# ToughStoneX/Self-Supervised-MVS

Hardware: AMD Instinct MI355X
Metric: depth-samples/sec (N=3, 640x512, D=192) (higher is better)
Workload: dtype f32

## Files before the change

### self-supervised-mvs_amd/_lib.py

```python
from __future__ import annotations

import ctypes as C
import os

_HERE = os.path.dirname(os.path.abspath(__file__))
LIB_PATH = os.path.join(_HERE, "libmvs_hip.so")

_f = C.c_void_p
_i = C.c_int
_ll = C.c_longlong
_s = C.c_void_p
_fl = C.c_float

class MvsUnetBlock(C.Structure):
    _fields_ = [("transposed", _i), ("stride", _i), ("src", _i), ("skip", _i), ("eps", _fl), ("momentum", _fl),
                ("cin", _i), ("cout", _i), ("d", _i), ("h", _i), ("w", _i)]


class MvsFeatBlock(C.Structure):
    _fields_ = [("cin", _i), ("cout", _i), ("ks", _i), ("stride", _i), ("eps", _fl), ("momentum", _fl), ("w_channels_last", _i),
                ("h", _i), ("w", _i)]


_pp = C.POINTER(C.c_void_p)
# ... 74 lines not shown
}

OP_CONV_FWD, OP_CONV_DGRAD, OP_CONV_WGRAD, OP_CONVT_FWD, OP_CONVT_DGRAD, OP_CONVT_WGRAD = range(6)


class MvsLib:

    def __init__(self, path: str = LIB_PATH, device_type: str = "cuda"):
        if not os.path.exists(path):
            raise RuntimeError(
                "libmvs_hip.so not found at %s -- build it with `python __graft_entry__.py` "
                "(hipcc --offload-arch=gfx950); there is no CPU / PyTorch fallback for the hot path" % path)
        self.path = path
        self.device_type = device_type
        self.cdll = C.CDLL(path)
        self.profiler = None
        for name, (res, args) in SIGNATURES.items():
            fn = getattr(self.cdll, name)
            fn.restype = res
            fn.argtypes = args
            setattr(self, "_" + name, fn)

    def call(self, name: str, *args, tag="", tstream=None):
        prof = self.profiler
        if prof is not None and (prof.names is None or name in prof.names):
            if not isinstance(tag, str):
                tag = tag[0] % tuple(tag[1:])
            if prof.wants(name, tag):
                import torch
                ev0, ev1 = torch.cuda.Event(enable_timing=True), torch.cuda.Event(enable_timing=True)
                ev0.record(tstream)
                rc = getattr(self, "_" + name)(*args)
                ev1.record(tstream)
                prof.add(name, tag, ev0, ev1)
                if rc != 0:
                    self._raise(name, rc)
                return
        rc = getattr(self, "_" + name)(*args)
        if rc != 0:
            self._raise(name, rc)

    def _raise(self, name, rc):
        msg = self._mvs_last_error().decode("utf-8", "replace")
        if rc in (-1, -2, -4):
            raise ValueError("%s failed (%d): %s" % (name, rc, msg))
        raise RuntimeError("%s failed (%d): %s" % (name, rc, msg))

    def raw(self, name: str, *args):
        return getattr(self, "_" + name)(*args)


_INSTANCE = None

DEFAULT_TUNING = {"k8": 7, "xcd": 1, "side_pre": 1, "conv_pers": 1, "conv_pers_min": 1024, "conv_pers_nw": 8, "wgrad_pers": 1, "conv_small": 1, "tr2pw": 1, "sweep_bwd": 0, "wgrad_small": 0, "wgrad_groups": 768, "wgrad8_groups": 192, "wgrad8_gs": 2, "wgrad8_nch": 2, "cout1_h4": 1, "wgrad2d_batch": 2048}


def get() -> MvsLib:
    global _INSTANCE
    if _INSTANCE is None:
        _INSTANCE = MvsLib()
        for item in filter(None, os.environ.get("MVS_TUNING", "").split(",")):
            key, _, val = item.partition("=")
            DEFAULT_TUNING[key.strip()] = int(val)
            _INSTANCE.call("mvs_set_tuning", key.strip().encode(), int(val))
    return _INSTANCE


class KernelTimer:

    def __init__(self, only=None, names=None):
        self.only = only
        self.names = names
        self.events = {}

    def wants(self, name, tag):
        return self.only is None or name in self.only or tag in self.only

    def add(self, name, tag, ev0, ev1):
        self.events.setdefault((name, tag), []).append((ev0, ev1))

    _REG_NAMES = frozenset(("mvs_conv3d_fwd", "mvs_convT3d_fwd", "mvs_conv3d_dgrad", "mvs_convT3d_dgrad", "mvs_conv3d_wgrad", "mvs_convT3d_wgrad",
                            "mvs_bn_relu_fwd_slots", "mvs_bn_relu_bwd_slots", "mvs_bn_bwd_reduce_slots", "mvs_conv3d_pack_weights_batch"))

    def allows_c_entry(self, lib, blocks):
        if self.names is None:
            return False
        hit = self.names & self._REG_NAMES
        if not hit:
            return True
        if not hit <= {"mvs_conv3d_wgrad", "mvs_convT3d_wgrad"} or self.only is None:
            return False
        want = [t for t in self.only if isinstance(t, str) and t.startswith("wgrad")]
        found = []
        for i, (transposed, cin, cout, stride, dims) in enumerate(blocks):
            tag = "%s:%d>%d:s%d:%dx%dx%dx%d" % (("wgradT" if transposed else "wgrad", cin, cout, stride) + tuple(dims))
            if tag in want:
                found.append((i, "mvs_convT3d_wgrad" if transposed else "mvs_conv3d_wgrad", tag))
        if len(found) != 1 or len(want) != 1:
            return False
        owner = getattr(lib, "_unet_timer", None)
        if owner is not self:
            if owner is not None:
                owner._harvest()
                owner._c = None
            lib.raw("mvs_unet_time_read", (C.c_float * 1024)(), 1024)
            lib.raw("mvs_unet_time_wgrad", found[0][0])
            lib._unet_timer = self
# ... 37 lines not shown
```

### self-supervised-mvs_amd/csrc/conv3d.hip

```cpp
#include "mvs_rt.h"
#include "conv_map.h"

int g_conv_cout1_d4 = 2;

extern int g_conv_split, g_conv_small, g_conv_small_wgs, g_conv_tr2pw;

#include "conv_args.h"

__device__ __forceinline__ void conv_pack_weights_item(const float* __restrict__ w, float* __restrict__ wp, int geom, int CC,
                                                       int Cin, int Cout, int NB, int layout, int flip, int idx) {
    const int j = idx & 3, lane = (idx >> 2) & 63;
    const int nb = (idx >> 8) % NB, kk = (idx >> 8) / NB;
    const int co = nb * 16 + (lane & 15);
    int ks, chunk = 0, cls = 0;
    if (geom == GEOM_TR2_PW) {
        int k0 = 0;
        for (cls = 0; cls < 4; ++cls) {
            int n = tr2p_ntaps(cls) * CC / 16;
            if (kk < k0 + n) break;
            k0 += n;
        }
        ks = kk - k0;
        const int kf = 16 * ks + 4 * (lane >> 4) + j;
        const int tp = kf / CC, cip = kf % CC, n = lane & 15, pw = n >> 3, cop = n & 7;
// ... 293 lines not shown
                const int f = wave * MB + mb;
                const int qd = qd0 + f / G::TQH, qh = qh0 + f % G::TQH;
                if (qd >= a.QD || qh >= a.QH) continue;
                const int od = qd * G::OS + pd_of(cls), oh = qh * G::OS + ph_of(cls);
#pragma unroll
                for (int r = 0; r < 4; ++r) {
                    const int qw = qw0 + 4 * g + r;
                    if (qw >= a.QW) continue;
                    const int ow = qw * G::OS + pw_of(cls);
                    const size_t obase = ((((size_t)b * a.Do + od) * a.Ho + oh) * a.Wo + ow) * a.Cout;
#pragma unroll
                    for (int nb = 0; nb < NB; ++nb) {
                        const int co = G::PW ? (l15 & 7) : (nb0 + nb) * 16 + l15;
                        if (co >= a.Cout) continue;
                        float v = acc[mb][nb][r];
                        float sv1 = v, sv2 = v * v;
                        if (a.scale) v = v * a.scale[co] + a.shift[co];
                        else if (a.shift) v = v + a.shift[co];
                        if (a.relu) v = fmaxf(v, 0.f);
                        if (SIDE && a.skip) v += SIDE_PRE ? skp[SIDE_PRE ? mb : 0][r][nb] : sk[e][r][nb];
                        if (SIDE && a.bn_raw) {
                            const float rw = SIDE_PRE ? rwp[SIDE_PRE ? mb : 0][r][nb] : rwv[e][r][nb];
                            sv1 = (rw * bsc[nb] + bsh[nb] > 0.f) ? v : 0.f;
                            sv2 = sv1 * ((rw - bmu[nb]) * bis[nb]);
                        }
                        st1[nb] += sv1;
                        st2[nb] += sv2;
                        a.y[obase + co] = v;
                    }
                }
            }
        }
    }

    if (a.slots) {
#pragma unroll
        for (int nb = 0; nb < NB; ++nb) {
            float s1 = st1[nb], s2 = st2[nb];
            s1 += __shfl_xor(s1, 16); s1 += __shfl_xor(s1, 32);
            s2 += __shfl_xor(s2, 16); s2 += __shfl_xor(s2, 32);
            if (G::PW) { s1 += __shfl_xor(s1, 8); s2 += __shfl_xor(s2, 8); }
            if (lane < 16) {
                red[((wave * NB + nb) * 16 + lane) * 2 + 0] = s1;
                red[((wave * NB + nb) * 16 + lane) * 2 + 1] = s2;
            }
        }
        __syncthreads();
        if (tid < 2 * NB * 16) {
            const int stat = tid / (NB * 16), n = tid % (NB * 16);
            if (nb0 * 16 + n < a.Cout) {
                float s = 0.f;
                for (int w = 0; w < 4; ++w) s += red[(w * NB * 16 + n) * 2 + stat];
                MVS_GLOBAL_ATOMIC_ADD_F64(a.slots + ((size_t)(blockIdx.x & (a.nslots - 1)) * 2 + stat) * a.Cout + nb0 * 16 + n, (double)s);
            }
        }
    }
}

template <int COUT, int VPT>
__global__ __launch_bounds__(256) void conv_cin1_kernel(const float* __restrict__ x, const float* __restrict__ wt,
                                                        float* __restrict__ y, int B, int D, int H, int W,
                                                        const float* __restrict__ bn_raw, const float* __restrict__ bn_stats,
                                                        double* __restrict__ slots, int nslots) {
    __shared__ float red[4 * 2 * COUT];
    const size_t total = (size_t)B * D * H * W;
    float sv[2 * COUT];
#pragma unroll
    for (int k = 0; k < 2 * COUT; ++k) sv[k] = 0.f;
#pragma unroll 1
    for (int it = 0; it < VPT; ++it) {
        const size_t v0 = ((size_t)blockIdx.x * VPT + it) * 256 + threadIdx.x;
        const bool live = v0 < total;
        const size_t v = live ? v0 : total - 1;
        const int w_ = (int)(v % W), h_ = (int)((v / W) % H), d_ = (int)((v / ((size_t)W * H)) % D);
        float4 rwq[COUT / 4];
#pragma unroll
        for (int q = 0; q < COUT / 4; ++q)
            rwq[q] = (slots && live) ? *reinterpret_cast<const float4*>(bn_raw + v * COUT + 4 * q) : make_float4(0.f, 0.f, 0.f, 0.f);
        int dofs[3], hofs[3], wofs[3];
        bool vd[3], vh[3], vw[3];
#pragma unroll
        for (int i = 0; i < 3; ++i) {
            const int d = d_ + i - 1, h = h_ + i - 1, w = w_ + i - 1;
            vd[i] = d >= 0 && d < D; vh[i] = h >= 0 && h < H; vw[i] = w >= 0 && w < W;
            dofs[i] = (min(max(d, 0), D - 1) - d_) * H * W;
            hofs[i] = (min(max(h, 0), H - 1) - h_) * W;
            wofs[i] = min(max(w, 0), W - 1) - w_;
        }
        const float* __restrict__ xc = x + v;
        float xv[27];
#pragma unroll
        for (int t = 0; t < 27; ++t) xv[t] = xc[dofs[t / 9] + hofs[(t / 3) % 3] + wofs[t % 3]];
        float acc[COUT];
#pragma unroll
        for (int c = 0; c < COUT; ++c) acc[c] = 0.f;
#pragma unroll
        for (int t = 0; t < 27; ++t) {
            const float xt = (vd[t / 9] && vh[(t / 3) % 3] && vw[t % 3]) ? xv[t] : 0.f;
#pragma unroll
            for (int c = 0; c < COUT; ++c) acc[c] = fmaf(xt, wt[t * COUT + c], acc[c]);
        }
        if (live) {
#pragma unroll
            for (int c = 0; c < COUT; c += 4)
                *reinterpret_cast<float4*>(y + v * COUT + c) = make_float4(acc[c], acc[c + 1], acc[c + 2], acc[c + 3]);
        }
// ... 824 lines not shown
                            const int bl = lane >> 2;
                            const int idx = BC ? ((4 * tg + (lane >> 4)) * 16 + (lane & 15)) * 8 + 4 * h + r
                                               : ((4 * tg + (bl >> 2)) * 16 + 4 * (bl & 3) + r) * 8 + (lane & 3) + 4 * h;
                            if (wv == 0) xt[idx] = acc[ch][tg][h][r];
                            else xt[idx] += acc[ch][tg][h][r];
                        }
            }
            __syncthreads();
        }
        for (int i = tid; i < 28 * 16 * 8; i += 256) {
            const int co = i & 7, cx = (i >> 3) & 15, tap = tapmap[i >> 7];
            if (tap < 27) a.part[(((size_t)blockIdx.x * 27 + tap) * a.CX + (chunk0 + ch) * 16 + cx) * 8 + co] = xt[i];
        }
    }
}

__global__ __launch_bounds__(256) void conv_wgrad_reduce_wide_kernel(const float* __restrict__ part, int nparts, int CX, int CG,
                                                                     float* __restrict__ gw) {
    __shared__ float red[16][17];
    const int n = 27 * CX * CG;
    const int el = threadIdx.x & 15, slice = threadIdx.x >> 4;
    const int e = blockIdx.x * 16 + el;
    const size_t stride = (size_t)n;
    float s0 = 0.f, s1 = 0.f, s2 = 0.f, s3 = 0.f;
    if (e < n) {
        int p = slice;
        for (; p + 48 < nparts; p += 64) {
            const float a0 = part[(size_t)p * stride + e], a1 = part[(size_t)(p + 16) * stride + e];
            const float a2 = part[(size_t)(p + 32) * stride + e], a3 = part[(size_t)(p + 48) * stride + e];
            s0 += a0; s1 += a1; s2 += a2; s3 += a3;
        }
        for (; p < nparts; p += 16) s0 += part[(size_t)p * stride + e];
    }
    red[slice][el] = (s0 + s1) + (s2 + s3);
    __syncthreads();
    if (slice == 0 && e < n) {
        float t = 0.f;
#pragma unroll
        for (int k = 0; k < 16; ++k) t += red[k][el];
        const int cg = e % CG, cx = (e / CG) % CX, tap = e / (CG * CX);
        gw[((size_t)cg * CX + cx) * 27 + tap] = t;
    }
}

static int pick_cc(int geom, int cin) {
    if (geom == GEOM_TR2) return cin;
    if (geom == GEOM_S2) return 8;
    return (cin % 16 == 0) ? 16 : 8;
}

int g_conv_cc_wide = 0;
int g_conv_cin1_vpt = 1;
static int pick_cc_k(int geom, int kgeom, int cin) {
    if (g_conv_cc_wide) {
        if (kgeom == GEOM_S1_SMALL && (cin == 32 || cin == 64)) return cin;
        if (kgeom == GEOM_S2_SMALL && (cin == 16 || cin == 32)) return cin;
    }
    return pick_cc(geom, cin);
}

static size_t packed_floats(int geom, int cin, int cout) {
    const int cc = pick_cc(geom, cin);
    int nb = mvs_cdiv(cout, 16);
    if (nb == 3) nb = 4;
    return (size_t)total_ksteps(geom, cin, cc) * nb * 256;
}

int g_conv_split = 1;
int g_conv_tr2pw = 1;
int g_conv_small_wgs = 384;
int g_conv_small = 1;
int g_conv_c8 = 7;
int g_conv_wgrad_groups = 768;
int g_conv_cout1_h4 = 1;
int g_conv_wgrad8_groups = 192;
int g_conv_wgrad8_nch = 2;
int g_conv_wgrad_small = 0;
int g_conv_side_pre = 1;
int g_conv_pers = 1;
int g_conv_pers_min_wgs = 1024;
int g_conv_wgrad_pers = 1;
bool conv_wgrad_pers_serves(int geom, int CX, int CG);
int run_conv_wgrad_pers(int geom, const WgradArgs& a, int max_groups, hipStream_t st);
bool conv_c8_wgrad_gs_serves(int geom, int CX, int CG);
int run_conv_c8_wgrad_gs(const WgradArgs& a, int max_groups, int waves, hipStream_t st);
int g_conv_wgrad8_gs = 2;
bool conv_pers_serves(int geom, int cin, int cout);
int run_conv_pers(int geom, const ConvArgs& a, hipStream_t st);
bool conv_x3_serves(int geom, const ConvArgs& a);
int run_conv_x3(const ConvArgs& a, const float* w, int wlayout, int flip, hipStream_t st);
bool conv_x3_fwd_serves(int geom, const ConvArgs& a);
int run_conv_x3_fwd(const ConvArgs& a, const float* w, int wlayout, int flip, float* ws, hipStream_t st);
extern int g_conv_x3;
int g_conv_xcd = 1;

template <int GEOM, int CC>
static int launch_igemm_nb(const ConvArgs& a, int NB, int nblocks, hipStream_t st) {
    dim3 grid(nblocks, a.nb_total / NB), block(256);
    if (a.skip || a.bn_raw) {
        switch (NB) {
            case 1:
                if (g_conv_side_pre) MVS_LAUNCH((conv_igemm_kernel<GEOM, CC, 1, 2>), grid, block, 0, st, a);
                else MVS_LAUNCH((conv_igemm_kernel<GEOM, CC, 1, 1>), grid, block, 0, st, a);
                break;
            case 2: MVS_LAUNCH((conv_igemm_kernel<GEOM, CC, 2, 1>), grid, block, 0, st, a); break;
            case 4: MVS_LAUNCH((conv_igemm_kernel<GEOM, CC, 4, 1>), grid, block, 0, st, a); break;
            default: mvs_set_error("conv igemm: Cout tile count %d unsupported", NB); return MVS_ERR_UNSUPPORTED;
        }
        return mvs_check_launch("conv_igemm");
    }
    switch (NB) {
        case 1: MVS_LAUNCH((conv_igemm_kernel<GEOM, CC, 1, 0>), grid, block, 0, st, a); break;
        case 2: MVS_LAUNCH((conv_igemm_kernel<GEOM, CC, 2, 0>), grid, block, 0, st, a); break;
        case 4: MVS_LAUNCH((conv_igemm_kernel<GEOM, CC, 4, 0>), grid, block, 0, st, a); break;
        default: mvs_set_error("conv igemm: Cout tile count %d unsupported", NB); return MVS_ERR_UNSUPPORTED;
    }
    return mvs_check_launch("conv_igemm");
}

static void igemm_tiling(int geom, int B, int QD, int QH, int QW, int cout, int& kgeom, int& NB, int& nblocks) {
    const int nb_total = mvs_cdiv(cout, 16) == 3 ? 4 : mvs_cdiv(cout, 16);
    nblocks = B * mvs_cdiv(QD, geom_tqd(geom)) * mvs_cdiv(QH, geom_tqh(geom)) * mvs_cdiv(QW, 16);
    NB = nb_total;
    if (g_conv_split && nblocks < 512 && NB > 1) NB = 1;
    kgeom = geom;
    const long thr = (long)g_conv_small_wgs * (geom == GEOM_S2 ? 24 : (geom == GEOM_S1 ? 3 : 1));
    if (g_conv_small == 2 || (g_conv_small == 1 && (long)nblocks * (nb_total / NB) < thr)) {
        kgeom = geom + GEOM_S1_SMALL;
        nblocks = B * mvs_cdiv(QD, geom_tqd(kgeom)) * mvs_cdiv(QH, geom_tqh(kgeom)) * mvs_cdiv(QW, 16);
    }
}

struct Epilogue {
    const float* scale; const float* shift; const float* skip; int relu;
    double* slots; int nslots;
    const float* bn_raw; const float* bn_stats;
};

struct IgemmPlan {
    int geom, wlayout, flip, B, Di, Hi, Wi, cin, cout;
    bool cin1;
};
enum { MVS_OP_CONV_FWD = 0, MVS_OP_CONV_DGRAD = 1, MVS_OP_CONV_WGRAD = 2,
       MVS_OP_CONVT_FWD = 3, MVS_OP_CONVT_DGRAD = 4, MVS_OP_CONVT_WGRAD = 5 };

static int check_stride(int stride, int D, int H, int W, const char* what) {
    MVS_REQUIRE(stride == 1 || stride == 2, MVS_ERR_UNSUPPORTED, "%s: stride must be 1 or 2, got %d", what, stride);
    MVS_REQUIRE(D > 0 && H > 0 && W > 0, MVS_ERR_SHAPE, "%s: bad spatial shape %dx%dx%d", what, D, H, W);
    return MVS_OK;
}

static int plan_for(int op, int B, int D, int H, int W, int Cin, int Cout, int stride, IgemmPlan& p, const char* what) {
    int rc = check_stride(stride, D, H, W, what);
    if (rc) return rc;
    MVS_REQUIRE(B > 0 && (long long)B * D * H * W * (stride == 2 ? 8 : 1) < (1LL << 31), MVS_ERR_SHAPE,
                "%s: %d x %d x %d x %d voxels do not fit the kernels' 32-bit voxel indices", what, B, D, H, W);
    p = {};
    p.B = B; p.cin1 = false;
    switch (op) {
        case MVS_OP_CONV_FWD:
            p.geom = stride == 2 ? GEOM_S2 : GEOM_S1; p.wlayout = WL_OIK; p.flip = 0;
            p.Di = D; p.Hi = H; p.Wi = W; p.cin = Cin; p.cout = Cout;
            return MVS_OK;
        case MVS_OP_CONV_DGRAD:
            p.cin = Cout; p.cout = Cin; p.wlayout = WL_IOK;
            if (stride == 1) {
                p.geom = GEOM_S1; p.flip = 1; p.Di = D; p.Hi = H; p.Wi = W;
                p.cin1 = Cout == 1;
            } else {
                MVS_REQUIRE(D % 2 == 0 && H % 2 == 0 && W % 2 == 0, MVS_ERR_SHAPE, "%s stride 2: D,H,W must be even", what);
                p.geom = GEOM_TR2; p.flip = 0; p.Di = D / 2; p.Hi = H / 2; p.Wi = W / 2;
            }
            return MVS_OK;
        case MVS_OP_CONVT_FWD:
            p.wlayout = WL_IOK; p.Di = D; p.Hi = H; p.Wi = W; p.cin = Cin; p.cout = Cout;
            if (stride == 1) { p.geom = GEOM_S1; p.flip = 1; } else { p.geom = GEOM_TR2; p.flip = 0; }
            return MVS_OK;
        case MVS_OP_CONVT_DGRAD:
            p.wlayout = WL_OIK; p.flip = 0; p.cin = Cout; p.cout = Cin;
            if (stride == 1) { p.geom = GEOM_S1; p.Di = D; p.Hi = H; p.Wi = W; }
            else { p.geom = GEOM_S2; p.Di = 2 * D; p.Hi = 2 * H; p.Wi = 2 * W; }
            return MVS_OK;
        default:
            mvs_set_error("%s: op %d has no weight image", what, op);
            return MVS_ERR_UNSUPPORTED;
    }
}

static void plan_grid(const IgemmPlan& p, int& QD, int& QH, int& QW) {
    if (p.geom == GEOM_S2) { QD = (p.Di - 1) / 2 + 1; QH = (p.Hi - 1) / 2 + 1; QW = (p.Wi - 1) / 2 + 1; }
    else { QD = p.Di; QH = p.Hi; QW = p.Wi; }
}
static bool plan_is_c8(const IgemmPlan& p, const Epilogue* ep) {
    return (g_conv_c8 & 3) && p.geom == GEOM_S1 && p.cout == 8 && (p.cin == 8 || p.cin == 16 || p.cin == 32) && !(ep && ep->bn_raw);
}
static bool plan_is_cout1(const IgemmPlan& p, const Epilogue* ep) {
    return p.geom == GEOM_S1 && p.cout == 1 && p.wlayout == WL_OIK && !p.flip && (p.cin == 8 || p.cin == 16) &&
           !(ep && (ep->slots || ep->bn_raw));
}

static int plan_pack(const IgemmPlan& p, const float* w, float* ws, PackItem& it) {
    it = {};
    it.w = w; it.wp = ws; it.kind = -1;
    if (p.cin1) {
        MVS_REQUIRE(p.cout == 8 || p.cout == 16, MVS_ERR_UNSUPPORTED, "conv3d_dgrad(Cout=1): Cin must be 8 or 16, got %d", p.cout);
        it.kind = 1; it.Cout = p.cout; it.total = 27 * p.cout;
        return MVS_OK;
    }
    MVS_REQUIRE(p.cin == 8 || p.cin == 16 || p.cin == 32 || p.cin == 64, MVS_ERR_UNSUPPORTED,
                "conv igemm: input channels must be 8/16/32/64, got %d", p.cin);
    MVS_REQUIRE(p.cout >= 1 && p.cout <= 64, MVS_ERR_UNSUPPORTED, "conv igemm: output channels must be <= 64, got %d", p.cout);
    MVS_REQUIRE(!(p.geom == GEOM_TR2 && p.cin < 16), MVS_ERR_UNSUPPORTED, "transposed stride-2 conv needs >= 16 input channels");
    int QD, QH, QW, kgeom, NB, nblocks;
    plan_grid(p, QD, QH, QW);
    igemm_tiling(p.geom, p.B, QD, QH, QW, p.cout, kgeom, NB, nblocks);
    const int cc = pick_cc_k(p.geom, kgeom, p.cin);
    const int nb_total = mvs_cdiv(p.cout, 16) == 3 ? 4 : mvs_cdiv(p.cout, 16);
    const int pgeom = (kgeom == GEOM_TR2 && cc == 16 && p.cout == 8 && g_conv_tr2pw) ? GEOM_TR2_PW : p.geom;
    it.kind = 0; it.geom = pgeom; it.CC = cc; it.Cin = p.cin; it.Cout = p.cout; it.NB = nb_total; it.layout = p.wlayout; it.flip = p.flip;
    it.total = (int)((size_t)total_ksteps(pgeom, p.cin, cc) * nb_total * 256);
    return MVS_OK;
}

static int launch_pack(const PackItem* items, int n, hipStream_t st) {
    for (int i0 = 0; i0 < n; i0 += MVS_PACK_BATCH_MAX) {
        PackBatch pb = {};
        int m = 0, maxtotal = 0;
        for (int i = i0; i < n && m < MVS_PACK_BATCH_MAX; ++i) {
            if (items[i].kind < 0) continue;
            pb.it[m++] = items[i];
            if (items[i].total > maxtotal) maxtotal = items[i].total;
        }
        if (m == 0) continue;
        MVS_LAUNCH(conv_pack_batch_kernel, dim3(mvs_cdiv(maxtotal, 256), m), dim3(256), 0, st, pb);
    }
    return mvs_check_launch("conv_pack_weights");
}

static int run_igemm(const IgemmPlan& p, const float* in, const float* wsrc, float* out, float* ws, const Epilogue& ep,
                     int ws_packed, hipStream_t st) {
    MVS_REQUIRE(in && wsrc && out && ws, MVS_ERR_NULL, "conv: null pointer argument");
    MVS_REQUIRE(!ep.slots || (ep.nslots >= 1 && ep.nslots <= 256 && (ep.nslots & (ep.nslots - 1)) == 0), MVS_ERR_SHAPE,
                "conv: statistic slot count must be a power of two <= 256, got %d", ep.nslots);
    MVS_REQUIRE(!ep.bn_raw || (ep.bn_stats && ep.slots), MVS_ERR_NULL, "conv: bn_raw needs bn_stats and slots");
    const int geom = p.geom, B = p.B, cin = p.cin, cout = p.cout;
    ConvArgs a = {};
    a.x = in; a.y = out; a.B = B; a.Di = p.Di; a.Hi = p.Hi; a.Wi = p.Wi; a.Cin = cin; a.Cout = cout;
    a.scale = ep.scale; a.shift = ep.shift; a.skip = ep.skip; a.relu = ep.relu;
    a.slots = ep.slots; a.nslots = ep.nslots; a.bn_raw = ep.bn_raw; a.bn_stats = ep.bn_stats;
    plan_grid(p, a.QD, a.QH, a.QW);
    if (geom == GEOM_S1) { a.Do = p.Di; a.Ho = p.Hi; a.Wo = p.Wi; }
    else if (geom == GEOM_S2) { a.Do = a.QD; a.Ho = a.QH; a.Wo = a.QW; }
    else { a.Do = 2 * p.Di; a.Ho = 2 * p.Hi; a.Wo = 2 * p.Wi; }
    a.ntd = mvs_cdiv(a.QD, geom_tqd(geom)); a.nth = mvs_cdiv(a.QH, geom_tqh(geom)); a.ntw = mvs_cdiv(a.QW, 16);
    if ((g_conv_x3 & 1) && conv_x3_serves(geom, a)) return run_conv_x3(a, wsrc, p.wlayout, p.flip, st);
    if ((g_conv_x3 & 2) && conv_x3_fwd_serves(geom, a)) return run_conv_x3_fwd(a, wsrc, p.wlayout, p.flip, ws, st);
    if (plan_is_c8(p, &ep)) {
        const int ntl = B * a.ntd * a.nth * a.ntw;
        const int nbc = ntl < 512 ? ntl : 512;
        if (cin == 32) MVS_LAUNCH((conv_c8_fwd_bc_kernel<16, 2>), dim3(nbc), dim3(256), 0, st, a, wsrc, p.wlayout, p.flip, g_conv_xcd);
        else if (cin == 16) MVS_LAUNCH((conv_c8_fwd_bc_kernel<16, 1>), dim3(nbc), dim3(256), 0, st, a, wsrc, p.wlayout, p.flip, g_conv_xcd);
        else MVS_LAUNCH((conv_c8_fwd_bc_kernel<8, 1>), dim3(nbc), dim3(256), 0, st, a, wsrc, p.wlayout, p.flip, g_conv_xcd);
        return mvs_check_launch("conv_c8_fwd_bc");
    }
    int nblocks = B * a.ntd * a.nth * a.ntw;
    if (plan_is_cout1(p, &ep)) {
        if (cin == 8 && g_conv_cout1_h4) {
            a.ntd = mvs_cdiv(a.QD, CO1_TD); a.nth = mvs_cdiv(a.QH, CO1_TH); a.ntw = mvs_cdiv(a.QW, CO1_TW);
            MVS_LAUNCH(conv_cout1_h4_kernel, dim3(B * a.ntd * a.nth * a.ntw), dim3(256), 0, st, a, wsrc);
        } else if (cin == 8) MVS_LAUNCH((conv_cout1_kernel<8>), dim3(nblocks), dim3(256), 0, st, a, wsrc);
        else MVS_LAUNCH((conv_cout1_kernel<16>), dim3(nblocks), dim3(256), 0, st, a, wsrc);
        return mvs_check_launch("conv_cout1");
    }
    int NB, kgeom;
    a.nb_total = mvs_cdiv(cout, 16) == 3 ? 4 : mvs_cdiv(cout, 16);
    igemm_tiling(geom, B, a.QD, a.QH, a.QW, cout, kgeom, NB, nblocks);
    const int cc = pick_cc_k(geom, kgeom, cin);
    a.ntd = mvs_cdiv(a.QD, geom_tqd(kgeom)); a.nth = mvs_cdiv(a.QH, geom_tqh(kgeom));
    if (!ws_packed) {
        PackItem it;
        int rc = plan_pack(p, wsrc, ws, it);
        if (rc) return rc;
        rc = launch_pack(&it, 1, st);
        if (rc) return rc;
    } else {
        MVS_REQUIRE(cin == 8 || cin == 16 || cin == 32 || cin == 64, MVS_ERR_UNSUPPORTED, "conv igemm: input channels must be 8/16/32/64, got %d", cin);
        MVS_REQUIRE(cout >= 1 && cout <= 64, MVS_ERR_UNSUPPORTED, "conv igemm: output channels must be <= 64, got %d", cout);
        MVS_REQUIRE(!(geom == GEOM_TR2 && cin < 16), MVS_ERR_UNSUPPORTED, "transposed stride-2 conv needs >= 16 input channels");
    }
    a.wp = ws;
    if (g_conv_pers && conv_pers_serves(geom, cin, cout) && (long)nblocks * (a.nb_total / NB) >= g_conv_pers_min_wgs) {
        a.ntd = mvs_cdiv(a.QD, geom_tqd(geom)); a.nth = mvs_cdiv(a.QH, geom_tqh(geom));
        return run_conv_pers(geom, a, st);
    }
    if ((g_conv_pers & 1) && kgeom == GEOM_TR2 && cc == 16 && cout == 8 && g_conv_tr2pw && conv_pers_serves(GEOM_TR2_PW, cin, cout) &&
        nblocks >= g_conv_pers_min_wgs)
        return run_conv_pers(GEOM_TR2_PW, a, st);
    if (kgeom == GEOM_S1) return cc == 16 ? launch_igemm_nb<GEOM_S1, 16>(a, NB, nblocks, st)
                                          : launch_igemm_nb<GEOM_S1, 8>(a, NB, nblocks, st);
    if (kgeom == GEOM_S2) return launch_igemm_nb<GEOM_S2, 8>(a, NB, nblocks, st);
    if (kgeom == GEOM_S1_SMALL) {
        if (cc == 64) return launch_igemm_nb<GEOM_S1_SMALL, 64>(a, NB, nblocks, st);
        if (cc == 32) return launch_igemm_nb<GEOM_S1_SMALL, 32>(a, NB, nblocks, st);
        return cc == 16 ? launch_igemm_nb<GEOM_S1_SMALL, 16>(a, NB, nblocks, st) : launch_igemm_nb<GEOM_S1_SMALL, 8>(a, NB, nblocks, st);
    }
    if (kgeom == GEOM_S2_SMALL) {
        if (cc == 32) return launch_igemm_nb<GEOM_S2_SMALL, 32>(a, NB, nblocks, st);
        if (cc == 16) return launch_igemm_nb<GEOM_S2_SMALL, 16>(a, NB, nblocks, st);
        return launch_igemm_nb<GEOM_S2_SMALL, 8>(a, NB, nblocks, st);
    }
    if (kgeom == GEOM_TR2_SMALL) {
        if (cc == 16) return launch_igemm_nb<GEOM_TR2_SMALL, 16>(a, NB, nblocks, st);
        if (cc == 32) return launch_igemm_nb<GEOM_TR2_SMALL, 32>(a, NB, nblocks, st);
        return launch_igemm_nb<GEOM_TR2_SMALL, 64>(a, NB, nblocks, st);
    }
    if (cc == 16 && cout == 8 && g_conv_tr2pw) return launch_igemm_nb<GEOM_TR2_PW, 16>(a, NB, nblocks, st);
    if (cc == 16) return launch_igemm_nb<GEOM_TR2, 16>(a, NB, nblocks, st);
    if (cc == 32) return launch_igemm_nb<GEOM_TR2, 32>(a, NB, nblocks, st);
    return launch_igemm_nb<GEOM_TR2, 64>(a, NB, nblocks, st);
}

static int run_cin1(const IgemmPlan& p, const float* gy, const float* w, float* gx, float* ws, const Epilogue& ep, int ws_packed,
                    hipStream_t st) {
    MVS_REQUIRE(gy && w && gx && ws, MVS_ERR_NULL, "conv3d_dgrad: null pointer argument");
    MVS_REQUIRE(!ep.skip, MVS_ERR_UNSUPPORTED, "conv3d_dgrad: the Cout = 1 input gradient takes no summand");
    MVS_REQUIRE(!ep.bn_raw || (ep.bn_stats && ep.slots), MVS_ERR_NULL, "conv3d_dgrad: bn_raw needs bn_stats and slots");
    MVS_REQUIRE(!ep.slots || (ep.bn_raw && ep.nslots >= 1 && ep.nslots <= 256 && (ep.nslots & (ep.nslots - 1)) == 0), MVS_ERR_SHAPE,
                "conv3d_dgrad: bad statistic slots");
    const int C = p.cout;
    if (!ws_packed) {
        PackItem it;
        int rc = plan_pack(p, w, ws, it);
        if (rc) return rc;
        rc = launch_pack(&it, 1, st);
        if (rc) return rc;
    } else {
        MVS_REQUIRE(C == 8 || C == 16, MVS_ERR_UNSUPPORTED, "conv3d_dgrad(Cout=1): Cin must be 8 or 16, got %d", C);
    }
    const size_t total = (size_t)p.B * p.Di * p.Hi * p.Wi;
    const int vpt = (g_conv_cin1_vpt == 5 || (g_conv_cin1_vpt == 4 && total >= (size_t)1 << 20)) ? 4 : 1;
    dim3 grid((unsigned)((total + 256 * vpt - 1) / (256 * vpt)));
    if (C == 8 && vpt == 4) MVS_LAUNCH((conv_cin1_kernel<8, 4>), grid, dim3(256), 0, st, gy, (const float*)ws, gx, p.B, p.Di, p.Hi, p.Wi, ep.bn_raw, ep.bn_stats, ep.slots, ep.nslots);
    else if (C == 8) MVS_LAUNCH((conv_cin1_kernel<8, 1>), grid, dim3(256), 0, st, gy, (const float*)ws, gx, p.B, p.Di, p.Hi, p.Wi, ep.bn_raw, ep.bn_stats, ep.slots, ep.nslots);
// ... 205 lines not shown
```

### self-supervised-mvs_amd/csrc/conv_map.h

```cpp
#pragma once

#if defined(__HIPCC__) || defined(MVS_CPU_EMUL)
#define MVS_HD __host__ __device__
#else
#define MVS_HD
#endif

enum { GEOM_S1 = 0, GEOM_S2 = 1, GEOM_TR2 = 2,
       GEOM_S1_SMALL = 3, GEOM_S2_SMALL = 4, GEOM_TR2_SMALL = 5,
       GEOM_TR2_PW = 6,
       GEOM_S1_DP = 7 };
enum { WL_OIK = 0, WL_IOK = 1 };

template <int GEOM>
struct ConvGeom;
template <>
struct ConvGeom<GEOM_S1> {
    static constexpr bool PW = false;
    static constexpr int BASE = GEOM_S1;
    static constexpr int TQD = 4, TQH = 4, TQW = 16, MB = 4;
    static constexpr int IS = 1, OS = 1, NCLS = 1, PAD = 1;
    static constexpr int RD = TQD + 2, RH = TQH + 2, RW = TQW + 2;
};
template <>
struct ConvGeom<GEOM_S1_DP> {
    static constexpr bool PW = false;
    static constexpr int BASE = GEOM_S1;
    static constexpr int TQD = 4, TQH = 4, TQW = 16, MB = 4;
    static constexpr int IS = 1, OS = 1, NCLS = 1, PAD = 1;
    static constexpr int RD = TQD + 2, RH = TQH + 2, RW = TQW + 2;
};
template <>
struct ConvGeom<GEOM_S2> {
    static constexpr bool PW = false;
    static constexpr int BASE = GEOM_S2;
    static constexpr int TQD = 2, TQH = 4, TQW = 16, MB = 2;
    static constexpr int IS = 2, OS = 1, NCLS = 1, PAD = 1;
    static constexpr int RD = 2 * TQD + 1, RH = 2 * TQH + 1, RW = 2 * TQW + 1;
};
template <>
struct ConvGeom<GEOM_TR2_PW> {
    static constexpr int BASE = GEOM_TR2;
    static constexpr bool PW = true;
    static constexpr int TQD = 4, TQH = 4, TQW = 16, MB = 4;
    static constexpr int IS = 1, OS = 2, NCLS = 4, PAD = 0;
    static constexpr int RD = TQD + 1, RH = TQH + 1, RW = TQW + 1;
};
template <>
struct ConvGeom<GEOM_TR2> {
    static constexpr bool PW = false;
    static constexpr int BASE = GEOM_TR2;
    static constexpr int TQD = 4, TQH = 4, TQW = 16, MB = 4;
    static constexpr int IS = 1, OS = 2, NCLS = 8, PAD = 0;
    static constexpr int RD = TQD + 1, RH = TQH + 1, RW = TQW + 1;
};
template <>
struct ConvGeom<GEOM_S1_SMALL> {
    static constexpr bool PW = false;
    static constexpr int BASE = GEOM_S1;
    static constexpr int TQD = 2, TQH = 2, TQW = 16, MB = 1;
    static constexpr int IS = 1, OS = 1, NCLS = 1, PAD = 1;
    static constexpr int RD = TQD + 2, RH = TQH + 2, RW = TQW + 2;
};
template <>
// ... 58 lines not shown
```

### self-supervised-mvs_amd/csrc/plane_sweep.hip

```cpp
#include <stdlib.h>
#include <string.h>
#include "mvs_rt.h"

#include <type_traits>
#include "plane_sweep_common.h"

template <int C, int NS_T>
__global__ __launch_bounds__(256) void plane_sweep_variance_fwd_kernel(SweepArgs a) {
    constexpr int QUADS = C / 4;
    constexpr int TW = Tile<C>::TW, TH = Tile<C>::TH;
    const int NS = NS_T > 0 ? NS_T : a.NS;
    const int tid = threadIdx.x;
    const int q = tid % QUADS, pl = tid / QUADS;
    const int x = (blockIdx.x % a.tiles_x) * TW + pl % TW, y = (blockIdx.x / a.tiles_x) * TH + pl / TW;
    const int b = blockIdx.z;
    if (x >= a.W || y >= a.H) return;
    const int HW = a.H * a.W, pix = y * a.W + x;
    const int d0 = blockIdx.y * a.dslab;
    const int d1 = min(a.D, d0 + a.dslab);
    const float xf = (float)x, yf = (float)y;
    const size_t fbase = (size_t)b * HW * C + 4 * q;
    const float4 r = ld4(a.ref + fbase + (size_t)pix * C);
    const float4 r2 = make_float4(r.x * r.x, r.y * r.y, r.z * r.z, r.w * r.w);
    const float inv_n = 1.0f / (float)(NS + 1);
// ... 1110 lines not shown
#pragma unroll
            for (int j = 0; j < 4; ++j) {
                jx0[j] = s_win[j][s][0]; jy0[j] = s_win[j][s][1];
                jw[j] = s_win[j][s][4] ? s_win[j][s][2] : 0; jh[j] = s_win[j][s][3];
            }
            float* gp = a.gsrc[s] + (size_t)b * HW * C;
            for (int i = tid; i < uw * uh * C; i += 256) {
                const int c = i % C, t = i / C;
                const int txl = ux0 + t % uw, tyl = uy0 + t / uw;
                float acc = 0.f;
#pragma unroll
                for (int j = 0; j < 4; ++j) {
                    const int lx = txl - jx0[j], ly = tyl - jy0[j];
                    if (lx >= 0 && lx < jw[j] && ly >= 0 && ly < jh[j])
                        acc += lds[(j * NS_T + s) * VIEW_FLOATS + (ly * jw[j] + lx) * C + c];
                }
                if (acc != 0.f) MVS_GLOBAL_ATOMIC_ADD(gp + ((size_t)tyl * a.W + txl) * C + c, acc);
            }
        }
        __syncthreads();
        ds = de;
    }
    if (!WARP_ONLY) {
        float* stage = wwin;
#pragma unroll
        for (int k = 0; k < V; ++k) *reinterpret_cast<float4*>(stage + pl * C + cq + CK * k) = gr[k];
        MVS_WAVE_SYNC();
        constexpr int PPW = Cfg::PPW;
        for (int i = lane; i < PPW * C; i += 64) {
            const int p = i / C, c = i % C;
            const int px = bx0 + p % BW, py = by0 + p / BW;
            const float val = stage[i];
            if (px < a.W && py < a.H && val != 0.f) MVS_GLOBAL_ATOMIC_ADD(a.gref + ((size_t)b * HW + (size_t)py * a.W + px) * C + c, val);
        }
    }
}

static int g_sweep_fwd_variant = -1;
static int sweep_fwd_variant() {
    if (g_sweep_fwd_variant < 0) {
        const char* e = getenv("MVS_SWEEP_FWD");
        g_sweep_fwd_variant = (e && e[0] >= '0' && e[0] <= '4') ? e[0] - '0' : 3;
    }
    return g_sweep_fwd_variant;
}
static int g_sweep_nt = 0;
static int g_sweep_tile_w = 0;
static int g_sweep_dslab = 0;
extern int g_conv_split;
extern int g_conv_small;
extern int g_conv_small_wgs;
extern int g_conv_tr2pw;
extern int g_conv_cc_wide;
extern int g_conv_cin1_vpt;
extern int g_conv_c8;
extern int g_conv_xcd;
extern int g_conv_x3;
extern int g_conv_side_pre;
extern int g_conv_pers, g_conv_pers_min_wgs, g_conv_pers_groups, g_conv_pers_nw, g_conv_wgrad_pers;
extern int g_conv_wgrad_small;
extern int g_conv_wgrad_groups;
extern int g_conv_wgrad8_groups;
extern int g_conv_wgrad8_gs;
extern int g_conv_wgrad8_nch;
extern int g_conv_cout1_d4;
extern int g_conv_bf16_dp;
extern int g_conv2d_s2_mfma;
extern int g_conv2d_pp;
extern int g_conv2d_wgrad_groups;
extern int g_conv2d_wgrad_batch_groups;
extern int g_conv_cout1_h4;
static int g_sweep_bwd_variant = 0;
static int g_sweep_bwd_cpt = 4;
static int g_sweep_bwd_pf = 0;
static int g_sweep_xcd = 0;
static int g_sweep_fwd_dl = 2;
static int g_sweep_bwd_gd = 2;
static int g_sweep_fwd_pt = 0;
static int g_sweep_bwd_gd34 = 0;
static int g_sweep_bwd_gpf = 0;
int g_sweep_bwd_nowin = 0;
int g_sweep_bwd_dslab = 0;
struct MvsKnob { const char* name; int* var; int lo, hi; };
static const MvsKnob* mvs_find_knob(const char* key) {
    static const MvsKnob knobs[] = {
        {"nt", &g_sweep_nt, 0, 1},           {"tile_w", &g_sweep_tile_w, 0, 256},   {"dslab", &g_sweep_dslab, 0, 1 << 20},
        {"conv_split", &g_conv_split, 0, 1}, {"conv_small", &g_conv_small, 0, 2}, {"conv_small_wgs", &g_conv_small_wgs, 0, 1 << 20}, {"tr2pw", &g_conv_tr2pw, 0, 1}, {"cc_wide", &g_conv_cc_wide, 0, 1}, {"cin1_vpt", &g_conv_cin1_vpt, 1, 5}, {"k8", &g_conv_c8, 0, 15},             {"cout1_d4", &g_conv_cout1_d4, 0, 3}, {"bf16_dp", &g_conv_bf16_dp, 0, 1}, {"conv2d_pp", &g_conv2d_pp, 0, 1},
        {"wgrad2d_groups", &g_conv2d_wgrad_groups, 0, 1 << 20}, {"wgrad2d_batch", &g_conv2d_wgrad_batch_groups, 1, 4096},                     {"conv2d_s2_mfma", &g_conv2d_s2_mfma, 0, 2},
        {"xcd", &g_conv_xcd, 0, 1}, {"side_pre", &g_conv_side_pre, 0, 1}, {"conv_pers", &g_conv_pers, 0, 1}, {"conv_pers_min", &g_conv_pers_min_wgs, 0, 1 << 30}, {"conv_pers_groups", &g_conv_pers_groups, 0, 4096}, {"conv_pers_nw", &g_conv_pers_nw, 4, 8}, {"wgrad_pers", &g_conv_wgrad_pers, 0, 1}, {"wgrad_small", &g_conv_wgrad_small, 0, 3}, {"wgrad_groups", &g_conv_wgrad_groups, 1, 768}, {"wgrad8_groups", &g_conv_wgrad8_groups, 1, 512}, {"wgrad8_gs", &g_conv_wgrad8_gs, 0, 2}, {"wgrad8_nch", &g_conv_wgrad8_nch, 1, 2}, {"cout1_h4", &g_conv_cout1_h4, 0, 1},          {"sweep_fwd", &g_sweep_fwd_variant, 0, 4}, {"sweep_bwd", &g_sweep_bwd_variant, 0, 1},
        {"bwd_dslab", &g_sweep_bwd_dslab, 0, 1 << 20}, {"bwd_nowin", &g_sweep_bwd_nowin, 0, 1}, {"bwd_cpt", &g_sweep_bwd_cpt, 4, 8}, {"bwd_pf", &g_sweep_bwd_pf, 0, 2}, {"bwd_gd", &g_sweep_bwd_gd, 0, 2}, {"bwd_gd34", &g_sweep_bwd_gd34, 0, 1}, {"fwd_pt", &g_sweep_fwd_pt, 0, 1}, {"bwd_gpf", &g_sweep_bwd_gpf, 0, 1}, {"fwd_dl", &g_sweep_fwd_dl, 0, 2}, {"sweep_xcd", &g_sweep_xcd, 0, 1}, {"conv0_x3", &g_conv_x3, 0, 3},
    };
    for (const MvsKnob& k : knobs)
        if (strcmp(key, k.name) == 0) return &k;
    return nullptr;
}
extern "C" int mvs_set_tuning(const char* key, int value) {
    MVS_REQUIRE(key, MVS_ERR_NULL, "mvs_set_tuning: null key");
    const MvsKnob* k = mvs_find_knob(key);
    if (!k) {
        mvs_set_error("mvs_set_tuning: unknown key '%s'", key);
        return MVS_ERR_UNSUPPORTED;
    }
    *k->var = value < k->lo ? k->lo : (value > k->hi ? k->hi : value);
    return MVS_OK;
}
extern "C" int mvs_get_tuning(const char* key, int* value) {
    MVS_REQUIRE(key && value, MVS_ERR_NULL, "mvs_get_tuning: null argument");
    const MvsKnob* k = mvs_find_knob(key);
    if (!k) {
        mvs_set_error("mvs_get_tuning: unknown key '%s'", key);
        return MVS_ERR_UNSUPPORTED;
    }
    *value = *k->var;
    return MVS_OK;
}

template <int C, int N, int CPT, bool BF>
static bool launch_fwd_pt(const SweepArgs& a, dim3 grid, hipStream_t st) {
    if constexpr ((64 / (C / CPT)) * N <= 64) {
        MVS_LAUNCH((plane_sweep_variance_fwd_pt_kernel<C, N, CPT, BF>), grid, dim3(256), 0, st, a);
        return true;
    } else {
        return false;
    }
}

template <int C>
static int launch_fwd(SweepArgs& a, hipStream_t st) {
    a.tiles_x = mvs_cdiv(a.W, Tile<C>::TW);
    a.tiles_y = mvs_cdiv(a.H, Tile<C>::TH);
    dim3 grid(a.tiles_x * a.tiles_y, mvs_cdiv(a.D, a.dslab), a.B), block(256);
    const int variant = sweep_fwd_variant();
    a.nt_store = g_sweep_nt;
    a.xcd = g_sweep_xcd;
    if (g_sweep_dslab > 0) a.dslab = g_sweep_dslab;
    if (!a.warp_only && variant >= 2 && (a.NS <= 4 || a.NS == 6) && !(variant == 4 && a.NS > 2)) {
        constexpr int CPT8 = C >= 16 ? 8 : 4;
        constexpr int CPT16 = C >= 32 ? 16 : CPT8;
        const bool c16 = variant == 4 && CPT16 == 16;
        const bool c8 = !c16 && variant >= 3 && CPT8 == 8 && a.NS <= 4;
// ... 292 lines not shown
```

Baseline: 212.7.

## Add halo-tiled MFMA conv kernel for small-grid stride-1/2 3D convs

Adds a new implicit-GEMM 3D conv kernel that stages a 3x(TW)x(16-row) input halo per 16-channel chunk in shared memory, with optional double buffering, and reuses it across all 27 taps. Weights are prefetched in a register ring. It is used in place of the existing 'small' path when the grid is small, Cin is a multiple of 16 up to 64, and Cout spans 2 or 4 tiles. The aim is more reuse of input loads and better occupancy on the low-resolution layers. In exchange it adds another kernel variant, a new packing/cc choice, and extra shared memory use per block.

```diff
diff --git a/self-supervised-mvs_amd/_lib.py b/self-supervised-mvs_amd/_lib.py
--- a/self-supervised-mvs_amd/_lib.py
+++ b/self-supervised-mvs_amd/_lib.py
@@ -150,7 +150,7 @@
 
 _INSTANCE = None
 
-DEFAULT_TUNING = {"k8": 7, "xcd": 1, "side_pre": 1, "conv_pers": 1, "conv_pers_min": 1024, "conv_pers_nw": 8, "wgrad_pers": 1, "conv_small": 1, "tr2pw": 1, "sweep_bwd": 0, "wgrad_small": 0, "wgrad_groups": 768, "wgrad8_groups": 192, "wgrad8_gs": 2, "wgrad8_nch": 2, "cout1_h4": 1, "wgrad2d_batch": 2048}
+DEFAULT_TUNING = {"k8": 7, "xcd": 1, "side_pre": 1, "conv_pers": 1, "conv_pers_min": 1024, "conv_pers_nw": 8, "wgrad_pers": 1, "conv_small": 1, "conv_hm": 1, "tr2pw": 1, "sweep_bwd": 0, "wgrad_small": 0, "wgrad_groups": 768, "wgrad8_groups": 192, "wgrad8_gs": 2, "wgrad8_nch": 2, "cout1_h4": 1, "wgrad2d_batch": 2048}
 
 
 def get() -> MvsLib:
diff --git a/self-supervised-mvs_amd/csrc/conv3d.hip b/self-supervised-mvs_amd/csrc/conv3d.hip
--- a/self-supervised-mvs_amd/csrc/conv3d.hip
+++ b/self-supervised-mvs_amd/csrc/conv3d.hip
@@ -369,6 +369,156 @@
                 float s = 0.f;
                 for (int w = 0; w < 4; ++w) s += red[(w * NB * 16 + n) * 2 + stat];
                 MVS_GLOBAL_ATOMIC_ADD_F64(a.slots + ((size_t)(blockIdx.x & (a.nslots - 1)) * 2 + stat) * a.Cout + nb0 * 16 + n, (double)s);
+            }
+        }
+    }
+}
+
+template <int BASE>
+struct HmGeom {
+    static constexpr int IS = BASE == GEOM_S2 ? 2 : 1;
+    static constexpr int RH = 15 * IS + 3;
+};
+template <int BASE, int NBT, int MB, int NBUF, int SIDE>
+__global__ __launch_bounds__(256) void conv_hm_kernel(ConvArgs a) {
+    constexpr int CC = 16, CCP = CC + 4, CQ = CC / 4;
+    constexpr int IS = HmGeom<BASE>::IS;
+    constexpr int WPB = 4 / NBT, TW = WPB * MB;
+    constexpr int RD = 3, RW = (TW - 1) * IS + 3, RH = HmGeom<BASE>::RH;
+    constexpr int NR = RD * RW * RH, NITEMS = NR * CQ, NIT = (NITEMS + 255) / 256;
+    constexpr int BUFF = NR * CCP;
+    constexpr int KS = 27, PD = 9;
+    __shared__ __attribute__((aligned(16))) float tile[NBUF * BUFF];
+    __shared__ float red[4 * 16 * 2];
+
+    const int tid = threadIdx.x, lane = tid & 63, wave = tid >> 6;
+    const int g = lane >> 4, l15 = lane & 15;
+    const int nb = wave % NBT, m0 = (wave / NBT) * MB;
+
+    int t = blockIdx.x;
+    const int tw = t % a.ntw; t /= a.ntw;
+    const int th = t % a.nth; t /= a.nth;
+    const int qd0 = t % a.QD; t /= a.QD;
+    const int b = t;
+    const int qh0 = th * 16, qw0 = tw * TW;
+    const int co = nb * 16 + l15;
+
+    float sk[MB][4], rwv[MB][4];
+    float bmu = 0.f, bis = 0.f, bsc = 0.f, bsh = 0.f;
+    auto obase_of = [&](int m, int r) {
+        const int oh = qh0 + 4 * g + r, ow = qw0 + m;
+        return ((((size_t)b * a.Do + qd0) * a.Ho + oh) * a.Wo + ow) * a.Cout;
+    };
+    auto valid = [&](int m, int r) { return qh0 + 4 * g + r < a.QH && qw0 + m < a.QW && co < a.Cout; };
+#pragma unroll
+    for (int m = 0; m < MB; ++m)
+#pragma unroll
+        for (int r = 0; r < 4; ++r) {
+            const bool ok = SIDE && valid(m0 + m, r);
+            sk[m][r] = (ok && a.skip) ? a.skip[obase_of(m0 + m, r) + co] : 0.f;
+            rwv[m][r] = (ok && a.bn_raw) ? a.bn_raw[obase_of(m0 + m, r) + co] : 0.f;
+        }
+    if (SIDE && a.bn_raw && co < a.Cout) {
+        bmu = a.bn_stats[co]; bis = a.bn_stats[a.Cout + co]; bsc = a.bn_stats[2 * a.Cout + co]; bsh = a.bn_stats[3 * a.Cout + co];
+    }
+
+    auto halo = [&](int chunk, float4 (&v)[NIT], int (&off)[NIT]) {
+        stage_load<NIT>(v, off, tid, NITEMS, [&](int i, const float*& src, int& o) {
+            const int vox = i / CQ, cq = i % CQ;
+            const int rw = vox % RW, rh = (vox / RW) % RH, rd = vox / (RW * RH);
+            const int id = qd0 * IS + rd - 1, ih = qh0 * IS + rh - 1, iw = qw0 * IS + rw - 1;
+            o = ((rd * RW + rw) * RH + rh) * CCP + 4 * cq;
+            if (id >= 0 && id < a.Di && ih >= 0 && ih < a.Hi && iw >= 0 && iw < a.Wi)
+                src = a.x + ((((size_t)b * a.Di + id) * a.Hi + ih) * a.Wi + iw) * a.Cin + chunk * CC + 4 * cq;
+        });
+    };
+    int baseA[MB];
+#pragma unroll
+    for (int m = 0; m < MB; ++m) baseA[m] = ((m0 + m) * IS * RH + l15 * IS) * CCP + 4 * g;
+    auto tapoff = [](int ks) { return (((ks / 9) * RW + ks % 3) * RH + (ks / 3) % 3) * CCP; };
+
+    const int nchunks = a.Cin / CC, K = nchunks * KS;
+    f32x4 acc[MB];
+#pragma unroll
+    for (int m = 0; m < MB; ++m) acc[m] = (f32x4){0.f, 0.f, 0.f, 0.f};
+    float4 hv[NIT];
+    int hoff[NIT];
+    halo(0, hv, hoff);
+    auto load_b = [&](int kk) {
+        const int kc = kk < K ? kk : K - 1;
+        return *reinterpret_cast<const float4*>(a.wp + (((size_t)kc * a.nb_total + nb) * 64 + lane) * 4);
+    };
+    float4 bq[PD];
+#pragma unroll
+    for (int u = 0; u < PD; ++u) bq[u] = load_b(u);
+
+    float4 af[MB];
+    for (int chunk = 0; chunk < nchunks; ++chunk) {
+        const int tb = NBUF == 2 ? (chunk & 1) * BUFF : 0;
+        if (NBUF == 1 && chunk > 0) __syncthreads();
+        stage_store<NIT>(&tile[tb], hv, hoff);
+        __syncthreads();
+        if (chunk + 1 < nchunks) halo(chunk + 1, hv, hoff);
+#pragma unroll
+        for (int m = 0; m < MB; ++m) af[m] = *reinterpret_cast<const float4*>(&tile[tb + baseA[m]]);
+        const int kk0 = chunk * KS;
+#pragma unroll
+        for (int ks = 0; ks < KS; ++ks) {
+            float4 an[MB];
+            const int ao = tb + tapoff(ks + 1 < KS ? ks + 1 : KS - 1);
+#pragma unroll
+            for (int m = 0; m < MB; ++m) an[m] = *reinterpret_cast<const float4*>(&tile[ao + baseA[m]]);
+            float4& bb = bq[ks % PD];
+#pragma unroll
+            for (int m = 0; m < MB; ++m) acc[m] = MVS_MFMA_16x16x4(af[m].x, bb.x, acc[m]);
+#pragma unroll
+            for (int m = 0; m < MB; ++m) acc[m] = MVS_MFMA_16x16x4(af[m].y, bb.y, acc[m]);
+#pragma unroll
+            for (int m = 0; m < MB; ++m) acc[m] = MVS_MFMA_16x16x4(af[m].z, bb.z, acc[m]);
+#pragma unroll
+            for (int m = 0; m < MB; ++m) acc[m] = MVS_MFMA_16x16x4(af[m].w, bb.w, acc[m]);
+            bb = load_b(kk0 + ks + PD);
+            MVS_SCHED_FENCE();
+#pragma unroll
+            for (int m = 0; m < MB; ++m) af[m] = an[m];
+        }
+    }
+
+    float st1 = 0.f, st2 = 0.f;
+#pragma unroll
+    for (int m = 0; m < MB; ++m)
+#pragma unroll
+        for (int r = 0; r < 4; ++r) {
+            if (!valid(m0 + m, r)) continue;
+            float v = acc[m][r];
+            float sv1 = v, sv2 = v * v;
+            if (a.scale) v = v * a.scale[co] + a.shift[co];
+            else if (a.shift) v = v + a.shift[co];
+            if (a.relu) v = fmaxf(v, 0.f);
+            if (SIDE && a.skip) v += sk[m][r];
+            if (SIDE && a.bn_raw) {
+                sv1 = (rwv[m][r] * bsc + bsh > 0.f) ? v : 0.f;
+                sv2 = sv1 * ((rwv[m][r] - bmu) * bis);
+            }
+            st1 += sv1;
+            st2 += sv2;
+            a.y[obase_of(m0 + m, r) + co] = v;
+        }
+
+    if (a.slots) {
+        st1 += __shfl_xor(st1, 16); st1 += __shfl_xor(st1, 32);
+        st2 += __shfl_xor(st2, 16); st2 += __shfl_xor(st2, 32);
+        if (lane < 16) {
+            red[(wave * 16 + lane) * 2 + 0] = st1;
+            red[(wave * 16 + lane) * 2 + 1] = st2;
+        }
+        __syncthreads();
+        if (tid < 2 * NBT * 16) {
+            const int stat = tid / (NBT * 16), n = tid % (NBT * 16);
+            if (n < a.Cout) {
+                float s = 0.f;
+                for (int w = n / 16; w < 4; w += NBT) s += red[(w * 16 + (n & 15)) * 2 + stat];
+                MVS_GLOBAL_ATOMIC_ADD_F64(a.slots + ((size_t)(blockIdx.x & (a.nslots - 1)) * 2 + stat) * a.Cout + n, (double)s);
             }
         }
     }
@@ -1299,6 +1449,7 @@
 int g_conv_cc_wide = 0;
 int g_conv_cin1_vpt = 1;
 static int pick_cc_k(int geom, int kgeom, int cin) {
+    if (kgeom == GEOM_S1_HM || kgeom == GEOM_S2_HM) return 16;
     if (g_conv_cc_wide) {
         if (kgeom == GEOM_S1_SMALL && (cin == 32 || cin == 64)) return cin;
         if (kgeom == GEOM_S2_SMALL && (cin == 16 || cin == 32)) return cin;
@@ -1365,7 +1516,15 @@
     return mvs_check_launch("conv_igemm");
 }
 
-static void igemm_tiling(int geom, int B, int QD, int QH, int QW, int cout, int& kgeom, int& NB, int& nblocks) {
+int g_conv_hm = 1;
+static int hm_mb(int kgeom, int nbt) { return (kgeom == GEOM_S2_HM && nbt == 2) ? 1 : 2; }
+static int hm_tw(int kgeom, int nbt) { return (4 / nbt) * hm_mb(kgeom, nbt); }
+static bool hm_serves(int geom, int cin, int nb_total, int QH, int QW) {
+    return g_conv_hm && (geom == GEOM_S1 || geom == GEOM_S2) && cin % 16 == 0 && cin <= 64 && (nb_total == 2 || nb_total == 4) &&
+           (long)QH * (mvs_cdiv(QW, 16) * 16) >= (long)QW * (mvs_cdiv(QH, 16) * 16);
+}
+
+static void igemm_tiling(int geom, int B, int QD, int QH, int QW, int cin, int cout, int& kgeom, int& NB, int& nblocks) {
     const int nb_total = mvs_cdiv(cout, 16) == 3 ? 4 : mvs_cdiv(cout, 16);
     nblocks = B * mvs_cdiv(QD, geom_tqd(geom)) * mvs_cdiv(QH, geom_tqh(geom)) * mvs_cdiv(QW, 16);
     NB = nb_total;
@@ -1375,7 +1534,30 @@
     if (g_conv_small == 2 || (g_conv_small == 1 && (long)nblocks * (nb_total / NB) < thr)) {
         kgeom = geom + GEOM_S1_SMALL;
         nblocks = B * mvs_cdiv(QD, geom_tqd(kgeom)) * mvs_cdiv(QH, geom_tqh(kgeom)) * mvs_cdiv(QW, 16);
-    }
+        if (g_conv_small == 1 && hm_serves(geom, cin, nb_total, QH, QW)) {
+            kgeom = geom == GEOM_S1 ? GEOM_S1_HM : GEOM_S2_HM;
+            NB = nb_total;
+            nblocks = B * QD * mvs_cdiv(QH, 16) * mvs_cdiv(QW, hm_tw(kgeom, nb_total));
+        }
+    }
+}
+
+template <int BASE, int NBT, int MB, int NBUF>
+static void launch_hm_t(const ConvArgs& a, dim3 grid, hipStream_t st) {
+    if (a.skip || a.bn_raw) MVS_LAUNCH((conv_hm_kernel<BASE, NBT, MB, NBUF, 1>), grid, dim3(256), 0, st, a);
+    else MVS_LAUNCH((conv_hm_kernel<BASE, NBT, MB, NBUF, 0>), grid, dim3(256), 0, st, a);
+}
+static int launch_hm(int kgeom, const ConvArgs& a, int nblocks, hipStream_t st) {
+    const dim3 grid(nblocks);
+    const bool db = a.Cin > 16;
+    if (kgeom == GEOM_S1_HM) {
+        if (a.nb_total == 4) { if (db) launch_hm_t<GEOM_S1, 4, 2, 2>(a, grid, st); else launch_hm_t<GEOM_S1, 4, 2, 1>(a, grid, st); }
+        else { if (db) launch_hm_t<GEOM_S1, 2, 2, 2>(a, grid, st); else launch_hm_t<GEOM_S1, 2, 2, 1>(a, grid, st); }
+    } else {
+        if (a.nb_total == 4) { if (db) launch_hm_t<GEOM_S2, 4, 2, 2>(a, grid, st); else launch_hm_t<GEOM_S2, 4, 2, 1>(a, grid, st); }
+        else { if (db) launch_hm_t<GEOM_S2, 2, 1, 2>(a, grid, st); else launch_hm_t<GEOM_S2, 2, 1, 1>(a, grid, st); }
+    }
+    return mvs_check_launch("conv_hm");
 }
 
 struct Epilogue {
@@ -1460,7 +1642,7 @@
     MVS_REQUIRE(!(p.geom == GEOM_TR2 && p.cin < 16), MVS_ERR_UNSUPPORTED, "transposed stride-2 conv needs >= 16 input channels");
     int QD, QH, QW, kgeom, NB, nblocks;
     plan_grid(p, QD, QH, QW);
-    igemm_tiling(p.geom, p.B, QD, QH, QW, p.cout, kgeom, NB, nblocks);
+    igemm_tiling(p.geom, p.B, QD, QH, QW, p.cin, p.cout, kgeom, NB, nblocks);
     const int cc = pick_cc_k(p.geom, kgeom, p.cin);
     const int nb_total = mvs_cdiv(p.cout, 16) == 3 ? 4 : mvs_cdiv(p.cout, 16);
     const int pgeom = (kgeom == GEOM_TR2 && cc == 16 && p.cout == 8 && g_conv_tr2pw) ? GEOM_TR2_PW : p.geom;
@@ -1521,7 +1703,7 @@
     }
     int NB, kgeom;
     a.nb_total = mvs_cdiv(cout, 16) == 3 ? 4 : mvs_cdiv(cout, 16);
-    igemm_tiling(geom, B, a.QD, a.QH, a.QW, cout, kgeom, NB, nblocks);
+    igemm_tiling(geom, B, a.QD, a.QH, a.QW, cin, cout, kgeom, NB, nblocks);
     const int cc = pick_cc_k(geom, kgeom, cin);
     a.ntd = mvs_cdiv(a.QD, geom_tqd(kgeom)); a.nth = mvs_cdiv(a.QH, geom_tqh(kgeom));
     if (!ws_packed) {
@@ -1536,6 +1718,10 @@
         MVS_REQUIRE(!(geom == GEOM_TR2 && cin < 16), MVS_ERR_UNSUPPORTED, "transposed stride-2 conv needs >= 16 input channels");
     }
     a.wp = ws;
+    if (kgeom == GEOM_S1_HM || kgeom == GEOM_S2_HM) {
+        a.ntd = a.QD; a.nth = mvs_cdiv(a.QH, 16); a.ntw = mvs_cdiv(a.QW, hm_tw(kgeom, a.nb_total));
+        return launch_hm(kgeom, a, nblocks, st);
+    }
     if (g_conv_pers && conv_pers_serves(geom, cin, cout) && (long)nblocks * (a.nb_total / NB) >= g_conv_pers_min_wgs) {
         a.ntd = mvs_cdiv(a.QD, geom_tqd(geom)); a.nth = mvs_cdiv(a.QH, geom_tqh(geom));
         return run_conv_pers(geom, a, st);
diff --git a/self-supervised-mvs_amd/csrc/conv_map.h b/self-supervised-mvs_amd/csrc/conv_map.h
--- a/self-supervised-mvs_amd/csrc/conv_map.h
+++ b/self-supervised-mvs_amd/csrc/conv_map.h
@@ -9,7 +9,8 @@
 enum { GEOM_S1 = 0, GEOM_S2 = 1, GEOM_TR2 = 2,
        GEOM_S1_SMALL = 3, GEOM_S2_SMALL = 4, GEOM_TR2_SMALL = 5,
        GEOM_TR2_PW = 6,
-       GEOM_S1_DP = 7 };
+       GEOM_S1_DP = 7,
+       GEOM_S1_HM = 8, GEOM_S2_HM = 9 };
 enum { WL_OIK = 0, WL_IOK = 1 };
 
 template <int GEOM>
diff --git a/self-supervised-mvs_amd/csrc/plane_sweep.hip b/self-supervised-mvs_amd/csrc/plane_sweep.hip
--- a/self-supervised-mvs_amd/csrc/plane_sweep.hip
+++ b/self-supervised-mvs_amd/csrc/plane_sweep.hip
@@ -1186,6 +1186,7 @@
 extern int g_conv_small_wgs;
 extern int g_conv_tr2pw;
 extern int g_conv_cc_wide;
+extern int g_conv_hm;
 extern int g_conv_cin1_vpt;
 extern int g_conv_c8;
 extern int g_conv_xcd;
@@ -1219,7 +1220,7 @@
 static const MvsKnob* mvs_find_knob(const char* key) {
     static const MvsKnob knobs[] = {
         {"nt", &g_sweep_nt, 0, 1},           {"tile_w", &g_sweep_tile_w, 0, 256},   {"dslab", &g_sweep_dslab, 0, 1 << 20},
-        {"conv_split", &g_conv_split, 0, 1}, {"conv_small", &g_conv_small, 0, 2}, {"conv_small_wgs", &g_conv_small_wgs, 0, 1 << 20}, {"tr2pw", &g_conv_tr2pw, 0, 1}, {"cc_wide", &g_conv_cc_wide, 0, 1}, {"cin1_vpt", &g_conv_cin1_vpt, 1, 5}, {"k8", &g_conv_c8, 0, 15},             {"cout1_d4", &g_conv_cout1_d4, 0, 3}, {"bf16_dp", &g_conv_bf16_dp, 0, 1}, {"conv2d_pp", &g_conv2d_pp, 0, 1},
+        {"conv_split", &g_conv_split, 0, 1}, {"conv_small", &g_conv_small, 0, 2}, {"conv_small_wgs", &g_conv_small_wgs, 0, 1 << 20}, {"tr2pw", &g_conv_tr2pw, 0, 1}, {"cc_wide", &g_conv_cc_wide, 0, 1}, {"conv_hm", &g_conv_hm, 0, 1}, {"cin1_vpt", &g_conv_cin1_vpt, 1, 5}, {"k8", &g_conv_c8, 0, 15},             {"cout1_d4", &g_conv_cout1_d4, 0, 3}, {"bf16_dp", &g_conv_bf16_dp, 0, 1}, {"conv2d_pp", &g_conv2d_pp, 0, 1},
         {"wgrad2d_groups", &g_conv2d_wgrad_groups, 0, 1 << 20}, {"wgrad2d_batch", &g_conv2d_wgrad_batch_groups, 1, 4096},                     {"conv2d_s2_mfma", &g_conv2d_s2_mfma, 0, 2},
         {"xcd", &g_conv_xcd, 0, 1}, {"side_pre", &g_conv_side_pre, 0, 1}, {"conv_pers", &g_conv_pers, 0, 1}, {"conv_pers_min", &g_conv_pers_min_wgs, 0, 1 << 30}, {"conv_pers_groups", &g_conv_pers_groups, 0, 4096}, {"conv_pers_nw", &g_conv_pers_nw, 4, 8}, {"wgrad_pers", &g_conv_wgrad_pers, 0, 1}, {"wgrad_small", &g_conv_wgrad_small, 0, 3}, {"wgrad_groups", &g_conv_wgrad_groups, 1, 768}, {"wgrad8_groups", &g_conv_wgrad8_groups, 1, 512}, {"wgrad8_gs", &g_conv_wgrad8_gs, 0, 2}, {"wgrad8_nch", &g_conv_wgrad8_nch, 1, 2}, {"cout1_h4", &g_conv_cout1_h4, 0, 1},          {"sweep_fwd", &g_sweep_fwd_variant, 0, 4}, {"sweep_bwd", &g_sweep_bwd_variant, 0, 1},
         {"bwd_dslab", &g_sweep_bwd_dslab, 0, 1 << 20}, {"bwd_nowin", &g_sweep_bwd_nowin, 0, 1}, {"bwd_cpt", &g_sweep_bwd_cpt, 4, 8}, {"bwd_pf", &g_sweep_bwd_pf, 0, 2}, {"bwd_gd", &g_sweep_bwd_gd, 0, 2}, {"bwd_gd34", &g_sweep_bwd_gd34, 0, 1}, {"fwd_pt", &g_sweep_fwd_pt, 0, 1}, {"bwd_gpf", &g_sweep_bwd_gpf, 0, 1}, {"fwd_dl", &g_sweep_fwd_dl, 0, 2}, {"sweep_xcd", &g_sweep_xcd, 0, 1}, {"conv0_x3", &g_conv_x3, 0, 3},
```

Result: faster. 215.3 (median of 6 runs) (+1.2%).
